# adeyemiadeoye/SelfConcordantSmoothOptimization.jl

Measured on AMD Instinct MI355X. Metric: iterate!() iterations/sec + achieved HBM GB/s, ProxGGNSCORE n=1M m=16k, higher is better.
Workload: dtype f64

## Files before the change

selfconcordantsmoothoptimization.jl_amd/csrc/gram.hip:

```cpp
#include <algorithm>
#include <cstdlib>
#include <type_traits>
#include <vector>

#include "common.h"

namespace scs {

}
#include "gram_strip.h"
namespace scs {

#define LDS_BARRIER()                                          \
  do {                                                         \
    asm volatile("s_waitcnt lgkmcnt(0)" ::: "memory");         \
    __builtin_amdgcn_s_barrier();                              \
    asm volatile("" ::: "memory");                             \
  } while (0)

__device__ __forceinline__ int bnd_claim(unsigned* ctr, int ntiles) {
  const int q8 = ntiles / 8, r8 = ntiles % 8;
  const int x0 = (int)((unsigned)__builtin_amdgcn_s_getreg((15 << 11) | 20) & 7u);
  for (int d = 0; d < 8; ++d) {
    const int x = (x0 + d) & 7, len = q8 + (x < r8 ? 1 : 0);
    if (len == 0) continue;
    const unsigned t = atomicAdd(ctr + x, 1u);
    if ((int)t < len) return x * q8 + (x < r8 ? x : r8) + (int)t;
  }
  return ntiles;
}
__device__ __forceinline__ int bnd_first(unsigned* ctr, unsigned skip, int ntiles, int* s) {
  if (threadIdx.x == 0) {
    const unsigned cu = ((unsigned)__builtin_amdgcn_s_getreg((31 << 11) | 4) >> 8) & 15u;
    const unsigned xcc = (unsigned)__builtin_amdgcn_s_getreg((15 << 11) | 20) & 7u;
    const unsigned xm = skip >> 24;
    const bool here = ((skip >> cu) & 1u) && (xm == 0 || ((xm >> xcc) & 1u));
    const unsigned arr = atomicAdd(ctr + 8, 1u);
    *s = (here && arr + 1 < gridDim.x) ? -1 : bnd_claim(ctr, ntiles);
  }
  __syncthreads();
  return *s;
}
__device__ __forceinline__ int bnd_next(unsigned* ctr, int ntiles, int* s) {
  __syncthreads();
  if (threadIdx.x == 0) *s = bnd_claim(ctr, ntiles);
  __syncthreads();
  return *s;
}

template <int TJC = 2>
__device__ __forceinline__ void gram_tile_store_row(const v4d (&acc)[4], int ti, int wr, int wc, int g, int fl,
                                                    int part, double* P, int GTI, int packed, int upper,
                                                    int accumulate, double* G, int64_t ldg, int tix, int bi, int bj) {
  auto addr = [&](int tj, int r) -> double* {
    const int il = wr * 64 + 16 * ti + g + 4 * r;
    const int jl = wc * 64 + 16 * tj + fl;
    if (part >= 0) return P + ((int64_t)part * GT + jl) * GTI + il;
    if (packed) return G + ((int64_t)tix * (GTI / GT) + il / GT) * GT * GT + jl * GT + (il % GT);
    if (upper) return G + ((int64_t)bi * GTI + il) * ldg + (int64_t)bj * GT + jl;
    return G + ((int64_t)bj * GT + jl) * ldg + (int64_t)bi * GTI + il;
  };
  if (accumulate && part < 0) {
#pragma unroll
// ... 404 lines not shown
  return hipGetLastError();
}

void gram_tile_list(int nb, int2* out, int* ntiles) {
  const int S = 8;
  const int nsb = (nb + S - 1) / S;
  int t = 0;
  for (int sbi = 0; sbi < nsb; ++sbi)
    for (int sbj = 0; sbj <= sbi; ++sbj)
      for (int i = sbi * S; i < (sbi + 1) * S && i < nb; ++i)
        for (int j = sbj * S; j < (sbj + 1) * S && j < nb; ++j)
          if (i >= j) out[t++] = make_int2(i, j);
  *ntiles = t;
}

void gram_tile_list_tall(int nb, int2* out, int* ntiles) {
  const int nbi = nb / 2, SI = 4, SJ = 8;
  int t = 0;
  for (int sbi = 0; sbi < (nbi + SI - 1) / SI; ++sbi)
    for (int sbj = 0; sbj <= sbi; ++sbj)
      for (int I = sbi * SI; I < (sbi + 1) * SI && I < nbi; ++I)
        for (int j = sbj * SJ; j < (sbj + 1) * SJ && j < nb; ++j)
          if (j <= 2 * I + 1) out[t++] = make_int2(I, j);
  *ntiles = t;
}

void gram_tile_list_rowmajor(int nb, int2* out) {
  int t = 0;
  for (int i = 0; i < nb; ++i)
    for (int j = 0; j <= i; ++j) out[t++] = make_int2(i, j);
}

hipError_t gram_launch_gen(const double* A1, int64_t lda1, const double* A2, int64_t lda2, const double* w,
                           int64_t k0, int64_t k1, const int2* tiles, int ntiles, double* G, int64_t ldg, int flags,
                           hipStream_t st);

template <int PIPE, int TI = 2, bool CM = false, bool AV = false, bool BND = false>
__global__ __launch_bounds__(128 * TI, (TI == 2 ? 2 : 1)) void gram_sia_kernel(
    const double* __restrict__ A, int64_t S, const double* __restrict__ w, int64_t k0, int64_t Nk,
    const int2* __restrict__ tiles, int ntiles, double* __restrict__ G, int64_t ldg, int flags,
    const int4* __restrict__ work, int seglen, int nsplit, double* __restrict__ P,
    const double* __restrict__ v, double* __restrict__ VP, int64_t vps, unsigned* __restrict__ scnt, int sob,
    const double* __restrict__ A2, int64_t S2) {
  static_assert(!(AV && CM), "the fused Aᵀv runs on the panel-blocked A only");
  constexpr int GTI = 64 * TI;
  constexpr int NT = 128 * TI;
  constexpr int FS = NT / 8;
  constexpr int NTI = 4;
  constexpr int NA = GTI / FS;
  constexpr int NB = GT / FS;
  constexpr int NMM = 2 * NTI * 4;
  constexpr int NRD = NTI + 4;
  constexpr int TAIL = NMM / 4;
  const int packed = flags & GRAM_PACKED, accumulate = flags & GRAM_ACCUMULATE, upper = flags & GRAM_UPPER;
  __shared__ __attribute__((aligned(16))) double lds[(GTI + GT) * GBK];
  const int orig = blockIdx.x;
  const int xcd = orig % 8;
  int bi, bj, tix, part = -1, piece = 0;
  __shared__ int s_claim;
  if constexpr (BND) {
    tix = bnd_first(scnt, (unsigned)sob, ntiles, &s_claim);
    if (tix < 0 || tix >= ntiles) return;
    bi = tiles[tix].x;
    bj = tiles[tix].y;
  } else if (work) {
    const int4 it = work[xcd * seglen + orig / 8];
    if (it.x < 0) return;
    bi = it.x;
    bj = it.y;
    tix = it.w;
    if (it.z >= 0) {
      piece = it.z;
      const int64_t L = ((Nk - k0 + (int64_t)nsplit * GBK - 1) / ((int64_t)nsplit * GBK)) * GBK;
      part = it.w;
      k0 = k0 + it.z * L;
      Nk = k0 + L < Nk ? k0 + L : Nk;
      if (Nk < k0) Nk = k0;
    }
  } else {
    const int q8 = ntiles / 8, r8 = ntiles % 8;
    tix = (xcd < r8 ? xcd * (q8 + 1) : r8 * (q8 + 1) + (xcd - r8) * q8) + orig / 8;
    const int2 tl = tiles[tix];
    bi = tl.x;
    bj = tl.y;
  }
bnd_tile:
  int tid_ = threadIdx.x;
  if constexpr (BND) asm volatile("" : "+v"(tid_));
  const int tid = tid_, lane = tid & 63, wid = tid >> 6;
  const int wr = wid >> 1, wc = wid & 1;
  const int sc = tid & 7, sf0 = tid >> 3;
  const int64_t st0 = k0 / GBK;
  const double* srcA = CM ? A + ((int64_t)bi * GTI + sf0) * S + k0 + 2 * sc
                          : A + ((int64_t)bi * (GTI / GT) * S + st0) * GT * GBK + sf0 * GBK + 2 * sc;
  const double* B2 = (CM && A2) ? A2 : A;
  const int64_t SB2 = (CM && A2) ? S2 : S;
  const double* srcB = CM ? B2 + ((int64_t)bj * GT + sf0) * SB2 + k0 + 2 * sc
                          : A + ((int64_t)bj * S + st0) * GT * GBK + sf0 * GBK + 2 * sc;
  const double* srcW = w + k0 + 2 * sc;
  const double* srcV = AV ? v + k0 + 2 * sc : nullptr;
  double* la = lds;
  double* lb = lds + GTI * GBK;
  int woff[NA];
#pragma unroll
  for (int i = 0; i < NA; ++i) {
    const int f = sf0 + FS * i;
    woff[i] = f * GBK + 2 * (sc ^ swz(f));
  }
  v2d ra[NA], rb[NB], rw, rv;
  double av[NB];
#pragma unroll
  for (int i = 0; i < NB; ++i) av[i] = 0.0;
  auto gload = [&](int64_t st, auto fa) {
    constexpr bool FA = decltype(fa)::value;
    if (PIPE == 3 && st >= 2) return;
    if (CM) {
#pragma unroll
      for (int i = 0; i < NA; ++i) ra[i] = *(const v2d*)(srcA + st * GBK + (int64_t)FS * i * S);
#pragma unroll
      for (int i = 0; i < NB; ++i) rb[i] = *(const v2d*)(srcB + st * GBK + (int64_t)FS * i * SB2);
    } else {
      const int64_t so = st * GT * GBK;
#pragma unroll
      for (int i = 0; i < NA; ++i) {
        const int f = FS * i;
        ra[i] = *(const v2d*)(srcA + so + (f >> 7) * S * GT * GBK + (f & 127) * GBK);
      }
#pragma unroll
      for (int i = 0; i < NB; ++i) rb[i] = *(const v2d*)(srcB + so + FS * GBK * i);
    }
    rw = *(const v2d*)(srcW + st * GBK);
    if (FA) rv = *(const v2d*)(srcV + st * GBK);
  };
  auto swrite = [&](auto fa) {
    constexpr bool FA = decltype(fa)::value;
#pragma unroll
    for (int i = 0; i < NA; ++i) *(v2d*)(la + woff[i]) = ra[i];
#pragma unroll
    for (int i = 0; i < NB; ++i) *(v2d*)(lb + woff[i]) = rb[i] * rw;
    if (FA) {
#pragma unroll
      for (int i = 0; i < NB; ++i) av[i] = __builtin_fma(rb[i][1], rv[1], __builtin_fma(rb[i][0], rv[0], av[i]));
    }
  };
  const int fl = lane & 15, g = lane >> 4, s = swz(fl);
  struct Frag {
    v2d a[NTI], b[4];
  };
  auto fread = [&](int p, Frag& F) {
    const int pc = ((4 * p + g) ^ s) * 2;
#pragma unroll
    for (int t = 0; t < NTI; ++t) F.a[t] = *(const v2d*)(la + (wr * 64 + 16 * t + fl) * GBK + pc);
#pragma unroll
    for (int t = 0; t < 4; ++t) F.b[t] = *(const v2d*)(lb + (wc * 64 + 16 * t + fl) * GBK + pc);
  };
  v4d acc[NTI][4];
#pragma unroll
  for (int i = 0; i < NTI; ++i)
#pragma unroll
    for (int j = 0; j < 4; ++j) acc[i][j] = (v4d){0.0, 0.0, 0.0, 0.0};
  auto mm = [&](const Frag& F, int n0, int n1) {
#pragma unroll
    for (int n = n0; n < n1; ++n) {
      const int u = n / (4 * NTI), ti = (n / 4) % NTI, tj = n & 3;
      acc[ti][tj] = __builtin_amdgcn_mfma_f64_16x16x4f64(F.a[ti][u], F.b[tj][u], acc[ti][tj], 0, 0, 0);
    }
  };
  auto barrier = [&]() {
    __builtin_amdgcn_sched_barrier(0);
    __builtin_amdgcn_s_waitcnt(0xC07F);
    __builtin_amdgcn_s_barrier();
    asm volatile("" ::: "memory");
    __builtin_amdgcn_sched_barrier(0);
  };
  const int nk = (int)((Nk - k0) / GBK);
  Frag F0, F1;
  auto run = [&](auto fa) {
    if (nk > 0) {
      gload(0, fa);
      swrite(fa);
      if (nk > 1) gload(1, fa);
      barrier();
      fread(0, F0);
    }
    auto body = [&](int k, bool has1, bool has2) {
      __builtin_amdgcn_sched_barrier(0);
      fread(1, F1);
      mm(F0, 0, NMM);
      if (PIPE) {
#pragma unroll
        for (int i = 0; i < NRD; ++i) {
          __builtin_amdgcn_sched_group_barrier(0x008, NMM / NRD, 0);
          __builtin_amdgcn_sched_group_barrier(0x100, 1, 0);
        }
      }
      barrier();
      if (has1) swrite(fa);
      if (has2) gload(k + 2, fa);
      mm(F1, 0, NMM - TAIL);
      if (PIPE) {
        if (has1) {
#pragma unroll
          for (int i = 0; i < NA + NB; ++i) {
            __builtin_amdgcn_sched_group_barrier(0x008, (NMM - TAIL) / (NA + NB), 0);
            __builtin_amdgcn_sched_group_barrier(0x200, 1, 0);
            if (has2) __builtin_amdgcn_sched_group_barrier(0x020, 1, 0);
          }
        }
        __builtin_amdgcn_sched_group_barrier(0x008, NMM, 0);
      }
      if (has1) {
        barrier();
        fread(0, F0);
      }
      mm(F1, NMM - TAIL, NMM);
      if (PIPE && has1) {
#pragma unroll
        for (int i = 0; i < NRD; ++i) {
          __builtin_amdgcn_sched_group_barrier(0x008, TAIL / NRD > 0 ? TAIL / NRD : 1, 0);
          __builtin_amdgcn_sched_group_barrier(0x100, 1, 0);
        }
      }
    };
    int k = 0;
    for (; k + 2 < nk; ++k) body(k, true, true);
    if (k + 1 < nk) {
      body(k, true, false);
      ++k;
    }
    if (k < nk) body(k, false, false);
  };
  const bool dav = AV && (int64_t)bj * GT / GTI == bi;
  if constexpr (AV) {
    if (dav) run(std::true_type{});
    else run(std::false_type{});
  } else {
    run(std::false_type{});
  }

  if (dav) {
#pragma unroll
    for (int i = 0; i < NB; ++i) {
      double t = av[i];
      t += __shfl_xor(t, 1);
      t += __shfl_xor(t, 2);
      t += __shfl_xor(t, 4);
      if (sc == 0) VP[(int64_t)piece * vps + (int64_t)bj * GT + sf0 + FS * i] = t;
    }
  }

  if constexpr (BND || CM) {
#pragma unroll
    for (int ti = 0; ti < NTI; ++ti)
      gram_tile_store_row(acc[ti], ti, wr, wc, g, fl, part, P, GTI, packed, upper, accumulate, G, ldg, tix, bi, bj);
  } else {
#pragma unroll
    for (int ti = 0; ti < NTI; ++ti)
#pragma unroll
      for (int tj = 0; tj < 4; ++tj)
#pragma unroll
        for (int r = 0; r < 4; ++r) {
          const int il = wr * 64 + 16 * ti + g + 4 * r;
          const int jl = wc * 64 + 16 * tj + fl;
          double* dst;
          if (part >= 0) {
            P[((int64_t)part * GT + jl) * GTI + il] = acc[ti][tj][r];
            continue;
          }
          if (packed) dst = G + ((int64_t)tix * (GTI / GT) + il / GT) * GT * GT + jl * GT + (il % GT);
          else if (upper) dst = G + ((int64_t)bi * GTI + il) * ldg + (int64_t)bj * GT + jl;
          else dst = G + ((int64_t)bj * GT + jl) * ldg + (int64_t)bi * GTI + il;
          if (accumulate) *dst += acc[ti][tj][r];
          else *dst = acc[ti][tj][r];
        }
  }
  if (!BND && scnt && part < 0) {
    __threadfence();
    __syncthreads();
    if (tid == 0) atomicAdd(scnt + bj / sob, 1u);
  }
  if constexpr (BND) {
    tix = bnd_next(scnt, ntiles, &s_claim);
    if (tix >= ntiles) return;
    bi = tiles[tix].x;
    bj = tiles[tix].y;
    goto bnd_tile;
  }
}

static int env_int(const char* name, int dflt) {
  const char* e = getenv(name);
  return e ? atoi(e) : dflt;
}
int gram_sia_mode() {
  static const int v = env_int("SCS_GRAM_SIA", 1);
  return v;
}
int gram_tall_mode() {
  static const int v = env_int("SCS_GRAM_GLDS", 3);
  return v;
}

int gram_fuse_ok(int tall) {
  const char* e = getenv("SCS_GRAM_FUSE");
  const int mode = e ? atoi(e) : 1;
  if (mode == 0 || (!tall && mode < 2)) return 0;
  return tall ? gram_tall_mode() == 3 : gram_sia_mode() == 1;
}

__global__ void gram_vfinal_kernel(const double* __restrict__ VP, int npiece, int64_t vps, int64_t m,
                                   double* __restrict__ out) {
  const int64_t f = (int64_t)blockIdx.x * blockDim.x + threadIdx.x;
  if (f >= m) return;
  double s = VP[f];
  for (int p = 1; p < npiece; ++p) s += VP[(int64_t)p * vps + f];
  out[f] = s;
}

hipError_t gram_vfinal_launch(const double* VP, int npiece, int64_t vps, int64_t m, double* out, hipStream_t st) {
  hipLaunchKernelGGL(gram_vfinal_kernel, dim3((unsigned)((m + 255) / 256)), dim3(256), 0, st, VP, npiece, vps, m, out);
  return hipGetLastError();
}

static thread_local const char* g_main_name = "";
const char* gram_main_kernel_name() { return g_main_name; }

hipError_t gram_launch(const double* A, int64_t lda, const double* w, int64_t Nk, const int2* tiles,
                       int ntiles, double* G, int64_t ldg, int packed, int tall, hipStream_t st, const double* v,
                       double* VP, int64_t vps) {
  if (ntiles <= 0) return hipSuccess;
  const int flags = ((packed & 1) ? GRAM_PACKED : GRAM_UPPER) | ((packed & 2) ? GRAM_ACCUMULATE : 0);
  if (v) {
    if (!gram_fuse_ok(tall)) return hipErrorInvalidValue;
    if (tall) {
      g_main_name = "gram_sia_kernel<1, 4, false, true, false>";
      hipLaunchKernelGGL((gram_sia_kernel<1, 4, false, true>), dim3(ntiles), dim3(512), 0, st, A, lda, w, (int64_t)0,
                         Nk, tiles, ntiles, G, ldg, flags, nullptr, 0, 0, nullptr, v, VP, vps, nullptr, 0, nullptr, (int64_t)0);
    } else {
      g_main_name = "gram_sia_kernel<1, 2, false, true, false>";
      hipLaunchKernelGGL((gram_sia_kernel<1, 2, false, true>), dim3(ntiles), dim3(256), 0, st, A, lda, w, (int64_t)0,
                         Nk, tiles, ntiles, G, ldg, flags, nullptr, 0, 0, nullptr, v, VP, vps, nullptr, 0, nullptr, (int64_t)0);
    }
    return hipGetLastError();
  }
  if (!tall && gram_sia_mode() == 0) {
    g_main_name = "gram_f64_kernel<false, 2, true, false>";
    hipLaunchKernelGGL((gram_f64_kernel<false, 2, true>), dim3(ntiles), dim3(256), 0, st, A, lda, A, lda, w,
                       (int64_t)0, Nk, tiles, ntiles, G, ldg, flags, nullptr, 0, 0, nullptr);
  } else if (!tall) {
    g_main_name = "gram_sia_kernel<1, 2, false, false, false>";
    hipLaunchKernelGGL((gram_sia_kernel<1, 2>), dim3(ntiles), dim3(256), 0, st, A, lda, w, (int64_t)0, Nk, tiles,
                       ntiles, G, ldg, flags, nullptr, 0, 0, nullptr, nullptr, nullptr, (int64_t)0, nullptr, 0, nullptr, (int64_t)0);
  } else if (gram_tall_mode() == 3) {
    g_main_name = "gram_sia_kernel<1, 4, false, false, false>";
    hipLaunchKernelGGL((gram_sia_kernel<1, 4>), dim3(ntiles), dim3(512), 0, st, A, lda, w, (int64_t)0, Nk, tiles,
                       ntiles, G, ldg, flags, nullptr, 0, 0, nullptr, nullptr, nullptr, (int64_t)0, nullptr, 0, nullptr, (int64_t)0);
  } else {
    g_main_name = "gram_glds_kernel<true, 1>";
    hipLaunchKernelGGL((gram_glds_kernel<true, 1>), dim3(ntiles), dim3(512), 0, st, A, lda, A, lda, w, (int64_t)0, Nk,
                       tiles, ntiles, G, ldg, flags, nullptr, 0, 0, nullptr);
  }
  return hipGetLastError();
}

template <int QC>
__global__ __launch_bounds__(256) void gram_small_kernel(const double* __restrict__ A1, int64_t lda1,
                                                         const double* A2, int64_t lda2,
                                                         const double* __restrict__ w, int64_t k0, int64_t Nk,
                                                         const int2* __restrict__ tiles, double* G, int64_t ldg,
                                                         int flags) {
  constexpr int NQ = GT / QC;
  __shared__ __attribute__((aligned(16))) double lds[2 * (GT + QC) * GBK];
  if (flags & GRAM_PRIO) __builtin_amdgcn_s_setprio(3);
  const int2 tl = tiles[blockIdx.x / NQ];
  const int64_t I0 = (int64_t)tl.x * GT, J0 = (int64_t)tl.y * GT + (blockIdx.x % NQ) * QC;
  double* Gt = (flags & GRAM_UPPER) ? G + I0 * ldg + J0 : G + J0 * ldg + I0;
  gram_small_strip<QC>(A1 + I0 * lda1, lda1, A2 + J0 * lda2, lda2, w, k0, Nk, Gt, ldg, flags, lds);
}

hipError_t gram_launch_small(const double* A1, int64_t lda1, const double* A2, int64_t lda2, const double* w,
                             int64_t k0, int64_t k1, const int2* tiles, int ntiles, double* G, int64_t ldg, int flags,
                             hipStream_t st) {
  if (ntiles <= 0) return hipSuccess;
  if ((k1 - k0) % (8 * GBK) != 0 || k1 <= k0) return hipErrorInvalidValue;
// ... 63 lines not shown
    hipLaunchKernelGGL((gram_sia_kernel<1, 2, true, false, true>), dim3(grid), dim3(256), 0, st, A1, lda1, w, k0, k1,
                       tiles, ntiles, G, ldg, flags, nullptr, 0, 0, nullptr, nullptr, nullptr, (int64_t)0, ctr,
                       (int)skip, nullptr, (int64_t)0);
  else if (gram_sia2(k1 - k0, lda2))
    hipLaunchKernelGGL((gram_sia_kernel<1, 2, true, false, true>), dim3(grid), dim3(256), 0, st, A1, lda1, w, k0, k1,
                       tiles, ntiles, G, ldg, flags, nullptr, 0, 0, nullptr, nullptr, nullptr, (int64_t)0, ctr,
                       (int)skip, A2, lda2);
  else
    hipLaunchKernelGGL((gram_f64_kernel<false, 2, false, true>), dim3(grid), dim3(256), 0, st, A1, lda1, A2, lda2, w,
                       k0, k1, tiles, ntiles, G, ldg, flags, nullptr, (int)skip, 0, reinterpret_cast<double*>(ctr));
  return hipGetLastError();
}

hipError_t gram_launch_ex(const double* A, int64_t lda, const double* w, int64_t k0, int64_t k1, const int2* tiles,
                          int ntiles, double* G, int64_t ldg, int accumulate, int noload, hipStream_t st) {
  const int flags = GRAM_UPPER | (accumulate ? GRAM_ACCUMULATE : 0);
  if (noload == 16 || noload == 17)
    hipLaunchKernelGGL((noload == 16 ? gram_sia_kernel<1, 4> : gram_sia_kernel<3, 4>), dim3(ntiles), dim3(512), 0,
                       st, A, (k1 - k0) / GBK, w, k0, k1, tiles, ntiles, G, ldg, flags, nullptr, 0, 0, nullptr, nullptr, nullptr, (int64_t)0, nullptr, 0, nullptr, (int64_t)0);
  else if (noload == 12)
    hipLaunchKernelGGL((gram_sia_kernel<3>), dim3(ntiles), dim3(256), 0, st, A, (k1 - k0) / GBK, w, k0, k1, tiles,
                       ntiles, G, ldg, flags, nullptr, 0, 0, nullptr, nullptr, nullptr, (int64_t)0, nullptr, 0, nullptr, (int64_t)0);
  else if (noload == 9 || noload == 10)
    hipLaunchKernelGGL((noload == 9 ? gram_sia_kernel<1> : gram_sia_kernel<0>), dim3(ntiles), dim3(256), 0, st, A,
                       (k1 - k0) / GBK, w, k0, k1, tiles, ntiles, G, ldg, flags, nullptr, 0, 0, nullptr, nullptr, nullptr, (int64_t)0, nullptr, 0, nullptr, (int64_t)0);
  else if (noload == 11)
    hipLaunchKernelGGL((gram_f64_kernel<false, 2, true>), dim3(ntiles), dim3(256), 0, st, A, (k1 - k0) / GBK, A,
                       (k1 - k0) / GBK, w, k0, k1, tiles, ntiles, G, ldg, flags, nullptr, 0, 0, nullptr);
  else if (noload == 7 || noload == 8)
    hipLaunchKernelGGL((noload == 7 ? gram_glds_kernel<true, 1> : gram_glds_kernel<true, 2>), dim3(ntiles), dim3(512),
                       0, st, A, (k1 - k0) / GBK, A, (k1 - k0) / GBK, w, k0, k1, tiles, ntiles, G, ldg, flags, nullptr,
                       0, 0, nullptr);
  else if (noload == 5)
    hipLaunchKernelGGL(gram_glds_kernel<true>, dim3(ntiles), dim3(512), 0, st, A, (k1 - k0) / GBK, A,
                       (k1 - k0) / GBK, w, k0, k1, tiles, ntiles, G, ldg, flags, nullptr, 0, 0, nullptr);
  else if (noload == 6)
    hipLaunchKernelGGL(gram_glds_kernel<false>, dim3(ntiles), dim3(512), 0, st, A, lda, A, lda, w, k0, k1, tiles,
                       ntiles, G, ldg, flags, nullptr, 0, 0, nullptr);
  else if (noload == 4)
    hipLaunchKernelGGL((gram_f64_kernel<true, 4>), dim3(ntiles), dim3(512), 0, st, A, lda, A, lda, w, k0, k1, tiles,
                       ntiles, G, ldg, flags, nullptr, 0, 0, nullptr);
  else if (noload == 3)
    hipLaunchKernelGGL((gram_f64_kernel<false, 4>), dim3(ntiles), dim3(512), 0, st, A, lda, A, lda, w, k0, k1, tiles,
                       ntiles, G, ldg, flags, nullptr, 0, 0, nullptr);
  else if (noload)
    hipLaunchKernelGGL((gram_f64_kernel<true, 2>), dim3(ntiles), dim3(256), 0, st, A, lda, A, lda, w, k0, k1, tiles,
                       ntiles, G, ldg, flags, nullptr, 0, 0, nullptr);
  else
    hipLaunchKernelGGL((gram_f64_kernel<false, 2>), dim3(ntiles), dim3(256), 0, st, A, lda, A, lda, w, k0, k1, tiles,
                       ntiles, G, ldg, flags, nullptr, 0, 0, nullptr);
  return hipGetLastError();
}

template <int TI>
__global__ void gram_combine_kernel(const double* __restrict__ P, const int4* __restrict__ items, int nsplit,
                                    double* __restrict__ G, int64_t ldg, int packed) {
  constexpr int GTI = 64 * TI;
  const int4 it = items[blockIdx.y];
  for (int e = blockIdx.x * blockDim.x + threadIdx.x; e < GTI * GT; e += gridDim.x * blockDim.x) {
    const int jl = e / GTI, il = e % GTI;
    double sum = 0.0;
    for (int sp = 0; sp < nsplit; ++sp) sum += P[(int64_t)(it.w + sp) * GTI * GT + e];
    double* dst = (packed & 1) ? G + ((int64_t)it.z * (GTI / GT) + il / GT) * GT * GT + jl * GT + (il % GT)
                               : G + ((int64_t)it.x * GTI + il) * ldg + (int64_t)it.y * GT + jl;
    if (packed & 2) *dst += sum;
    else *dst = sum;
  }
}

hipError_t gram_launch_sched(const double* A, int64_t lda, const double* w, int64_t Nk, const int4* work, int seglen,
                             int nsplit, const int4* comb, int ncomb, double* P, double* G, int64_t ldg, int packed,
                             int tall, hipStream_t st, const double* v, double* VP, int64_t vps, unsigned* scnt,
                             int sob) {
  if (scnt && !(gram_fuse_ok(tall) || (tall ? gram_tall_mode() == 3 : gram_sia_mode() == 1)))
    return hipErrorInvalidValue;
  const int flags = ((packed & 1) ? GRAM_PACKED : GRAM_UPPER) | ((packed & 2) ? GRAM_ACCUMULATE : 0);
  const int glds = gram_tall_mode();
  if (v && !gram_fuse_ok(tall)) return hipErrorInvalidValue;
  if (v && tall) {
    g_main_name = "gram_sia_kernel<1, 4, false, true, false>";
    hipLaunchKernelGGL((gram_sia_kernel<1, 4, false, true>), dim3(8 * seglen), dim3(512), 0, st, A, lda, w,
                       (int64_t)0, Nk, nullptr, 0, G, ldg, flags, work, seglen, nsplit, P, v, VP, vps, scnt, sob, nullptr, (int64_t)0);
  } else if (v) {
    g_main_name = "gram_sia_kernel<1, 2, false, true, false>";
    hipLaunchKernelGGL((gram_sia_kernel<1, 2, false, true>), dim3(8 * seglen), dim3(256), 0, st, A, lda, w,
                       (int64_t)0, Nk, nullptr, 0, G, ldg, flags, work, seglen, nsplit, P, v, VP, vps, scnt, sob, nullptr, (int64_t)0);
  } else if (tall && glds == 3) {
    g_main_name = "gram_sia_kernel<1, 4, false, false, false>";
    hipLaunchKernelGGL((gram_sia_kernel<1, 4>), dim3(8 * seglen), dim3(512), 0, st, A, lda, w, (int64_t)0, Nk,
                       nullptr, 0, G, ldg, flags, work, seglen, nsplit, P, nullptr, nullptr, (int64_t)0, scnt, sob, nullptr, (int64_t)0);
  } else if (tall && glds == 2) {
    g_main_name = "gram_glds_kernel<true, 1>";
    hipLaunchKernelGGL((gram_glds_kernel<true, 1>), dim3(8 * seglen), dim3(512), 0, st, A, lda, A, lda, w, (int64_t)0,
                       Nk, nullptr, 0, G, ldg, flags, work, seglen, nsplit, P);
  } else if (tall && glds == 1) {
    g_main_name = "gram_glds_kernel<true, 0>";
    hipLaunchKernelGGL(gram_glds_kernel<true>, dim3(8 * seglen), dim3(512), 0, st, A, lda, A, lda, w, (int64_t)0, Nk,
                       nullptr, 0, G, ldg, flags, work, seglen, nsplit, P);
  } else if (tall) {
    g_main_name = "gram_f64_kernel<false, 4, true, false>";
    hipLaunchKernelGGL((gram_f64_kernel<false, 4, true>), dim3(8 * seglen), dim3(512), 0, st, A, lda, A, lda, w,
                       (int64_t)0, Nk, nullptr, 0, G, ldg, flags, work, seglen, nsplit, P);
  } else if (gram_sia_mode() == 1) {
    g_main_name = "gram_sia_kernel<1, 2, false, false, false>";
    hipLaunchKernelGGL((gram_sia_kernel<1, 2>), dim3(8 * seglen), dim3(256), 0, st, A, lda, w, (int64_t)0, Nk, nullptr,
                       0, G, ldg, flags, work, seglen, nsplit, P, nullptr, nullptr, (int64_t)0, scnt, sob, nullptr, (int64_t)0);
  } else if (gram_sia_mode() == 2) {
    g_main_name = "gram_sia_kernel<0, 2, false, false, false>";
    hipLaunchKernelGGL((gram_sia_kernel<0>), dim3(8 * seglen), dim3(256), 0, st, A, lda, w, (int64_t)0, Nk, nullptr, 0,
                       G, ldg, flags, work, seglen, nsplit, P, nullptr, nullptr, (int64_t)0, scnt, sob, nullptr, (int64_t)0);
  } else {
    g_main_name = "gram_f64_kernel<false, 2, true, false>";
    hipLaunchKernelGGL((gram_f64_kernel<false, 2, true>), dim3(8 * seglen), dim3(256), 0, st, A, lda, A, lda, w,
                       (int64_t)0, Nk, nullptr, 0, G, ldg, flags, work, seglen, nsplit, P);
  }
  if (ncomb > 0) {
    if (tall)
      hipLaunchKernelGGL(gram_combine_kernel<4>, dim3(16, ncomb), dim3(256), 0, st, P, comb, nsplit, G, ldg, packed);
    else
      hipLaunchKernelGGL(gram_combine_kernel<2>, dim3(16, ncomb), dim3(256), 0, st, P, comb, nsplit, G, ldg, packed);
  }
  return hipGetLastError();
}

__global__ void strip_wait_kernel(const unsigned* __restrict__ cnt, unsigned target, int* __restrict__ flag) {
  if (threadIdx.x != 0) return;
  const uint64_t t0 = __builtin_amdgcn_s_memrealtime();
  while (__hip_atomic_load(cnt, __ATOMIC_ACQUIRE, __HIP_MEMORY_SCOPE_AGENT) < target) {
    __builtin_amdgcn_s_sleep(16);
    if (__builtin_amdgcn_s_memrealtime() - t0 > 3000000000ull) {
      __hip_atomic_store(flag, 1, __ATOMIC_RELAXED, __HIP_MEMORY_SCOPE_AGENT);
      break;
    }
  }
}

hipError_t strip_wait_launch(const unsigned* cnt, unsigned target, int* flag, hipStream_t st) {
  hipLaunchKernelGGL(strip_wait_kernel, dim3(1), dim3(64), 0, st, cnt, target, flag);
  return hipGetLastError();
}

hipError_t gram_launch_sched_cm(const double* X, int64_t ld, const double* w, int64_t k0, int64_t k1, const int4* work,
                                int seglen, int nsplit, const int4* comb, int ncomb, double* P, double* G, int64_t ldg,
                                int flags, hipStream_t st) {
  if (seglen <= 0 || k1 <= k0) return hipSuccess;
  hipLaunchKernelGGL((gram_sia_kernel<1, 2, true>), dim3(8 * seglen), dim3(256), 0, st, X, ld, w, k0, k1, nullptr, 0,
                     G, ldg, flags | GRAM_UPPER, work, seglen, nsplit, P, nullptr, nullptr, (int64_t)0, nullptr, 0, nullptr, (int64_t)0);
  if (ncomb > 0)
    hipLaunchKernelGGL(gram_combine_kernel<2>, dim3(16, ncomb), dim3(256), 0, st, P, comb, nsplit, G, ldg,
                       (flags & GRAM_ACCUMULATE) ? 2 : 0);
  return hipGetLastError();
}

int gram_schedule(const int2* tiles, int ntiles, int slots_per_xcd, std::vector<int4>& work, std::vector<int4>& comb,
                  int* nsplit, int* npart, int diag_first_gti) {
  const int q = ntiles / 8, r = ntiles % 8;
  int tail_max = 0;
  for (int x = 0; x < 8; ++x) {
    const int n = q + (x < r ? 1 : 0);
    const int t = n % slots_per_xcd;
    tail_max = std::max(tail_max, t);
  }
  int S = 1;
  if (tail_max > 0 && 4 * tail_max < 3 * slots_per_xcd)
    S = std::max(2, std::min(16, slots_per_xcd / tail_max));
  std::vector<std::vector<int4>> seg(8);
  comb.clear();
  int pslot = 0, t0 = 0;
  for (int x = 0; x < 8; ++x) {
    const int n = q + (x < r ? 1 : 0);
    const int tail = (S > 1) ? n % slots_per_xcd : 0;
    for (int i = 0; i < n - tail; ++i) {
      const int2 tl = tiles[t0 + i];
      seg[x].push_back(make_int4(tl.x, tl.y, -1, t0 + i));
    }
    if (diag_first_gti > 0)
      std::stable_partition(seg[x].begin(), seg[x].end(), [&](const int4& it) {
        return it.x == (int)((int64_t)it.y * GT / diag_first_gti);
      });
    for (int i = n - tail; i < n; ++i) {
      const int2 tl = tiles[t0 + i];
      comb.push_back(make_int4(tl.x, tl.y, t0 + i, pslot));
      for (int sp = 0; sp < S; ++sp) seg[x].push_back(make_int4(tl.x, tl.y, sp, pslot + sp));
      pslot += S;
    }
    t0 += n;
  }
  size_t seglen = 0;
  for (auto& v : seg) seglen = std::max(seglen, v.size());
  work.assign(8 * seglen, make_int4(-1, -1, -1, -1));
  for (int x = 0; x < 8; ++x)
    for (size_t i = 0; i < seg[x].size(); ++i) work[x * seglen + i] = seg[x][i];
  *nsplit = S;
  *npart = pslot;
  return (int)seglen;
}

hipError_t gram_unpack_launch(const double* P, const int2* tiles, int ntiles, double* G, int64_t ldg,
                              hipStream_t st) {
  if (ntiles <= 0) return hipSuccess;
  hipLaunchKernelGGL(gram_packx_kernel<true>, dim3(4, ntiles), dim3(256), 0, st, P, G, tiles, ldg);
  return hipGetLastError();
}

}
```

selfconcordantsmoothoptimization.jl_amd/csrc/gram_strip.h:

```cpp
#pragma once
#include "common.h"

namespace scs {

constexpr int GT = 128;
enum { GRAM_PACKED = 1, GRAM_ACCUMULATE = 2, GRAM_UPPER = 4, GRAM_PRIO = 8 };
constexpr int GBK = 16;

__device__ __forceinline__ int swz(int f) { return (f >> 1) & 7; }

template <int TJ>
__device__ __forceinline__ void gram_strip_store(const v4d (&acc)[2][TJ], double* Gt, int64_t ldg, int wr, int g,
                                                 int fl, int accumulate, int upper) {
  double* dst[2][TJ][4];
#pragma unroll
  for (int ti = 0; ti < 2; ++ti)
#pragma unroll
    for (int tj = 0; tj < TJ; ++tj)
#pragma unroll
      for (int r = 0; r < 4; ++r) {
        const int64_t I = wr * 32 + 16 * ti + g + 4 * r;
        const int64_t J = 16 * tj + fl;
        dst[ti][tj][r] = upper ? Gt + I * ldg + J : Gt + J * ldg + I;
      }
  if (accumulate) {
    double old[2][TJ][4];
#pragma unroll
    for (int ti = 0; ti < 2; ++ti)
#pragma unroll
      for (int tj = 0; tj < TJ; ++tj)
#pragma unroll
        for (int r = 0; r < 4; ++r) old[ti][tj][r] = *dst[ti][tj][r];
#pragma unroll
    for (int ti = 0; ti < 2; ++ti)
#pragma unroll
      for (int tj = 0; tj < TJ; ++tj)
#pragma unroll
        for (int r = 0; r < 4; ++r) *dst[ti][tj][r] = old[ti][tj][r] + acc[ti][tj][r];
  } else {
#pragma unroll
    for (int ti = 0; ti < 2; ++ti)
#pragma unroll
      for (int tj = 0; tj < TJ; ++tj)
#pragma unroll
        for (int r = 0; r < 4; ++r) *dst[ti][tj][r] = acc[ti][tj][r];
  }
}

template <int QC>
__device__ __forceinline__ void gram_small_strip(const double* __restrict__ Ai, int64_t lda1, const double* Aj,
                                                 int64_t lda2, const double* __restrict__ w, int64_t k0, int64_t Nk,
                                                 double* Gt, int64_t ldg, int flags, double* lds) {
  constexpr int RING = 8;
  constexpr int NQ = GT / QC;
  constexpr int TJ = QC / 16;
  constexpr int SBQ = (GT + QC) * GBK;
  (void)NQ;
  const int accumulate = flags & GRAM_ACCUMULATE, upper = flags & GRAM_UPPER;
  const int tid = threadIdx.x, lane = tid & 63, wr = tid >> 6;
// ... 63 lines not shown
```

selfconcordantsmoothoptimization.jl_amd/csrc/kernels.h:

```cpp
#pragma once
#include <hip/hip_runtime.h>
#include <stdint.h>

#include <vector>
#include "../../include/scsopt.h"

namespace scs {

struct ProxArgsH {
  int reg = 0;
  int use_prox = 1;
  double lam = 0.0, lam2 = 0.0;
  const double* lb = nullptr;
  const double* ub = nullptr;
  const int* gstart = nullptr;
  const int* gend = nullptr;
  const double* gw = nullptr;
  int ngroups = 0;
  const int* gmap = nullptr;
};

void gram_tile_list(int nb, int2* out, int* ntiles);
void gram_tile_list_tall(int nb, int2* out, int* ntiles);
const char* gram_main_kernel_name();
hipError_t gram_launch(const double* A, int64_t lda, const double* w, int64_t Nk, const int2* tiles, int ntiles,
                       double* G, int64_t ldg, int packed, int tall, hipStream_t st, const double* v = nullptr,
                       double* VP = nullptr, int64_t vps = 0);
int gram_fuse_ok(int tall);
hipError_t gram_vfinal_launch(const double* VP, int npiece, int64_t vps, int64_t m, double* out, hipStream_t st);
void gram_tile_list_rowmajor(int nb, int2* out);
hipError_t gram_launch_gen(const double* A1, int64_t lda1, const double* A2, int64_t lda2, const double* w,
                           int64_t k0, int64_t k1, const int2* tiles, int ntiles, double* G, int64_t ldg, int flags,
                           hipStream_t st);
hipError_t gram_launch_work_cm(const double* A1, int64_t lda1, const double* A2, int64_t lda2, const double* w,
                               int64_t K, const int4* work, int seglen, int nsplit, double* P, hipStream_t st);
hipError_t gram_launch_bounded(const double* A1, int64_t lda1, const double* A2, int64_t lda2, const double* w,
                               int64_t k0, int64_t k1, const int2* tiles, int ntiles, double* G, int64_t ldg, int flags,
                               unsigned* ctr, unsigned skip, int slots, hipStream_t st, bool zeroed = false);
hipError_t gram_launch_small(const double* A1, int64_t lda1, const double* A2, int64_t lda2, const double* w,
                             int64_t k0, int64_t k1, const int2* tiles, int ntiles, double* G, int64_t ldg, int flags,
                             hipStream_t st);
int gram_schedule(const int2* tiles, int ntiles, int slots_per_xcd, std::vector<int4>& work, std::vector<int4>& comb,
                  int* nsplit, int* npart, int diag_first_gti = 0);
hipError_t gram_launch_sched(const double* A, int64_t lda, const double* w, int64_t Nk, const int4* work, int seglen,
                             int nsplit, const int4* comb, int ncomb, double* P, double* G, int64_t ldg, int packed,
                             int tall, hipStream_t st, const double* v = nullptr, double* VP = nullptr,
                             int64_t vps = 0, unsigned* scnt = nullptr, int sob = 0);
hipError_t strip_wait_launch(const unsigned* cnt, unsigned target, int* flag, hipStream_t st);
hipError_t gram_pack_launch(const double* G, int64_t ldg, const int2* tiles, int ntiles, double* P, hipStream_t st);
hipError_t gram_unpack_launch(const double* P, const int2* tiles, int ntiles, double* G, int64_t ldg,
                              hipStream_t st);

struct DagTask {
  int64_t a1, a2, out;
  int32_t lda1, a1w;
  int32_t k0, nk;
  int32_t wneg, flags;
  int32_t dep0, ndep;
  int32_t sig0, sig1;
};
struct DagDep {
  int32_t c, target;
};
struct DagList {
  int t0 = 0, nt = 0;
  unsigned gen = 0;
};

struct CholAux {
  double* w = nullptr;
  int2* rect = nullptr;
  hipStream_t st2 = nullptr;
  hipStream_t stc = nullptr;
  hipStream_t st2h = nullptr;
  hipEvent_t ev1 = nullptr, ev2 = nullptr, ev3 = nullptr, ev4 = nullptr, ev0 = nullptr, ev5 = nullptr;
  int nblk = 0;
  unsigned* bctr = nullptr;
  int2* sbl = nullptr;
  unsigned bskip = 0;
  int bslots = 0;
  mutable int bslot = 0;
  mutable int chain_mode = 0;
  double* sscr = nullptr;
  struct StripSched {
    int4* work = nullptr;
    int seglen = 0, nsplit = 1;
    int4* comb = nullptr;
    int ncomb = 0;
  };
  std::vector<StripSched> ssched;
  double* spart = nullptr;
  unsigned* sflags = nullptr;
  int* serr = nullptr;
  unsigned sgen = 0;
  mutable bool no_persist = false;
  mutable bool no_dag = false;
// ... 235 lines not shown
```

selfconcordantsmoothoptimization.jl_amd/csrc/scsopt.cpp:

```cpp
#include <hip/hip_runtime.h>
#include <rccl/rccl.h>

#include <dlfcn.h>
#include <execinfo.h>
#include <signal.h>

#include <algorithm>
#include <chrono>
#include <cmath>
#include <cstdarg>
#include <cstddef>
#include <cstdio>
#include <cstdlib>
#include <cstring>
#include <limits>
#include <atomic>
#include <condition_variable>
#include <functional>
#include <memory>
#include <mutex>
#include <string>
#include <thread>
#include <utility>
#include <vector>
// ... 545 lines not shown
  c->nval = epilogue_blocks(c->Npad);
  c->nchunk = c->sparse ? c->bcsc.nblk : gemv_t_chunks(c->Npad);
  dfree_t(c, c->zpart);
  dfree_t(c, c->z);
  dfree_t(c, c->gN);
  dfree_t(c, c->hN);
  dfree_t(c, c->wN);
  dfree_t(c, c->vN);
  dfree_t(c, c->valpart);
  dfree_t(c, c->tpart);
  c->zpart = dalloc<double>(c, (size_t)c->nsplit * c->Npad);
  c->z = dalloc<double>(c, c->Npad);
  c->gN = dalloc<double>(c, c->Npad);
  c->hN = dalloc<double>(c, c->Npad);
  c->wN = dalloc<double>(c, c->Npad);
  c->vN = dalloc<double>(c, c->Npad);
  c->valpart = dalloc<double>(c, c->nval);
  c->tpart = dalloc<double>(c, (size_t)c->nchunk * c->mpad);
}

void ensure_gram(scs_ctx* c) {
  if (c->G) return;
  const int64_t mp = c->mpad;
  c->G = dalloc<double>(c, (size_t)mp * mp);
  c->Gc = dalloc<double>(c, (size_t)mp * mp);
  const int nb = (int)(mp / 128);
  std::vector<int2> tl((size_t)nb * (nb + 1) / 2 + nb), ul;
  int nt = 0;
  const char* sq = std::getenv("SCS_GRAM_TALL");
  c->tall = (nb % 2 == 0) && nb >= 96 && !(sq && sq[0] == '0');
  if (sq && sq[0] == '1') c->tall = (nb % 2 == 0);
  if (c->tall) {
    gram_tile_list_tall(nb, tl.data(), &nt);
    ul.resize(2 * (size_t)nt);
    for (int t = 0; t < nt; ++t) {
      ul[2 * t] = make_int2(2 * tl[t].x, tl[t].y);
      ul[2 * t + 1] = make_int2(2 * tl[t].x + 1, tl[t].y);
    }
  } else {
    gram_tile_list(nb, tl.data(), &nt);
    ul.assign(tl.begin(), tl.begin() + nt);
  }
  c->tiles = dalloc<int2>(c, nt);
  HCK(hipMemcpyAsync(c->tiles, tl.data(), sizeof(int2) * nt, hipMemcpyHostToDevice, c->st));
  c->ntiles = nt;
  c->nslots = (int)ul.size();
  {
    const char* ev = std::getenv("SCS_GRAM_SCHED");
    if (!(ev && ev[0] == '0')) {
      std::vector<int4> wk, cb;
      int npart = 0;
      const char* df = std::getenv("SCS_GRAM_DIAGFIRST");
      const int dfg = (df && df[0] == '0') ? 0 : c->tall ? 256 : (df && df[0] == '1') ? 128 : 0;
      c->gseglen = gram_schedule(tl.data(), nt, 32 * (c->tall ? 1 : 2), wk, cb, &c->gnsplit, &npart, dfg);
      c->gncomb = (int)cb.size();
      c->gwork = dalloc<int4>(c, wk.size());
      HCK(hipMemcpyAsync(c->gwork, wk.data(), sizeof(int4) * wk.size(), hipMemcpyHostToDevice, c->st));
      if (c->gncomb > 0) {
        c->gcomb = dalloc<int4>(c, cb.size());
        HCK(hipMemcpyAsync(c->gcomb, cb.data(), sizeof(int4) * cb.size(), hipMemcpyHostToDevice, c->st));
        c->gpart = dalloc<double>(c, (size_t)npart * (c->tall ? 256 : 128) * 128);
      }
    }
  }
  {
    const int OB = chol_outer_block(), ns = (nb + OB - 1) / OB;
    c->gstrip.assign(ns, scs_ctx::GStrip());
    c->vpieces = std::max(c->gnsplit, 1);
    int npart_max = 0;
    for (int s2 = 0; s2 < ns; ++s2) {
      std::vector<int2> st;
      for (int t = 0; t < nt; ++t)
        if (tl[t].y / OB == s2) st.push_back(tl[t]);
      std::vector<int4> wk, cb;
      int nsplit = 1, npart = 0;
      scs_ctx::GStrip& g = c->gstrip[s2];
      g.seglen = gram_schedule(st.data(), (int)st.size(), 32 * (c->tall ? 1 : 2), wk, cb, &nsplit, &npart);
      g.nsplit = nsplit;
      g.ncomb = (int)cb.size();
      g.work = dalloc<int4>(c, wk.size());
      HCK(hipMemcpyAsync(g.work, wk.data(), sizeof(int4) * wk.size(), hipMemcpyHostToDevice, c->st));
      if (!cb.empty()) {
        g.comb = dalloc<int4>(c, cb.size());
        HCK(hipMemcpyAsync(g.comb, cb.data(), sizeof(int4) * cb.size(), hipMemcpyHostToDevice, c->st));
      }
      npart_max = std::max(npart_max, npart);
      c->vpieces = std::max(c->vpieces, nsplit);
    }
    {
      const int slots = 32 * (c->tall ? 1 : 2);
      std::vector<std::vector<int4>> seg(8);
      c->gp_target.assign(ns, 0u);
      std::vector<int4> cbl;
      int nsplit = 1, npart = 0;
      for (int s2 = 0; s2 < ns; ++s2) {
        std::vector<int2> st;
        std::vector<int> ix;
        for (int t = 0; t < nt; ++t)
          if (tl[t].y / OB == s2) {
            st.push_back(tl[t]);
            ix.push_back(t);
          }
        const int n = (int)st.size();
        if (s2 + 1 < ns) {
          c->gp_target[s2] = (unsigned)n;
          const int q = n / 8, r = n % 8;
          int t0 = 0;
// ... 3589 lines not shown
```

Measured before the change: 0.2560.

## Skip redundant lower-half MFMA work on symmetric diagonal Gram tiles in tall mode

In the tall (TI=4) Gram kernel, tiles where bj == 2*bi+1 straddle the diagonal, so half of the 256x128 output block is a redundant copy of the other half. For those tiles the waves covering that half (wid<4) now skip their LDS fragment reads and MFMAs but still take part in global loads, LDS writes and barriers, and the A-panel rows shared with B are not reloaded. The host scheduler is reworked to place these cheaper tiles separately and spread them evenly across XCDs. Correctness relies on the epilogue mirroring or ignoring the skipped half, which is not visible here.

Measured after the change: 0.2580, median of 6. No clear change (+0.8%).

```diff
diff --git a/selfconcordantsmoothoptimization.jl_amd/csrc/gram.hip b/selfconcordantsmoothoptimization.jl_amd/csrc/gram.hip
--- a/selfconcordantsmoothoptimization.jl_amd/csrc/gram.hip
+++ b/selfconcordantsmoothoptimization.jl_amd/csrc/gram.hip
@@ -9,6 +9,7 @@
 
 }
 #include "gram_strip.h"
+#include "gram_schedule.h"
 namespace scs {
 
 #define LDS_BARRIER()                                          \
@@ -519,6 +520,8 @@
   constexpr int NMM = 2 * NTI * 4;
   constexpr int NRD = NTI + 4;
   constexpr int TAIL = NMM / 4;
+  constexpr int NA0 = GT / FS;
+  constexpr bool SYMM_OK = TI == 4 && !CM && !BND;
   const int packed = flags & GRAM_PACKED, accumulate = flags & GRAM_ACCUMULATE, upper = flags & GRAM_UPPER;
   __shared__ __attribute__((aligned(16))) double lds[(GTI + GT) * GBK];
   const int orig = blockIdx.x;
@@ -578,18 +581,19 @@
   double av[NB];
 #pragma unroll
   for (int i = 0; i < NB; ++i) av[i] = 0.0;
-  auto gload = [&](int64_t st, auto fa) {
+  auto gload = [&](int64_t st, auto fa, auto dt) {
     constexpr bool FA = decltype(fa)::value;
+    constexpr int IA0 = decltype(dt)::value ? NA0 : 0;
     if (PIPE == 3 && st >= 2) return;
     if (CM) {
 #pragma unroll
-      for (int i = 0; i < NA; ++i) ra[i] = *(const v2d*)(srcA + st * GBK + (int64_t)FS * i * S);
+      for (int i = IA0; i < NA; ++i) ra[i] = *(const v2d*)(srcA + st * GBK + (int64_t)FS * i * S);
 #pragma unroll
       for (int i = 0; i < NB; ++i) rb[i] = *(const v2d*)(srcB + st * GBK + (int64_t)FS * i * SB2);
     } else {
       const int64_t so = st * GT * GBK;
 #pragma unroll
-      for (int i = 0; i < NA; ++i) {
+      for (int i = IA0; i < NA; ++i) {
         const int f = FS * i;
         ra[i] = *(const v2d*)(srcA + so + (f >> 7) * S * GT * GBK + (f & 127) * GBK);
       }
@@ -599,10 +603,11 @@
     rw = *(const v2d*)(srcW + st * GBK);
     if (FA) rv = *(const v2d*)(srcV + st * GBK);
   };
-  auto swrite = [&](auto fa) {
+  auto swrite = [&](auto fa, auto dt) {
     constexpr bool FA = decltype(fa)::value;
-#pragma unroll
-    for (int i = 0; i < NA; ++i) *(v2d*)(la + woff[i]) = ra[i];
+    constexpr int IA0 = decltype(dt)::value ? NA0 : 0;
+#pragma unroll
+    for (int i = IA0; i < NA; ++i) *(v2d*)(la + woff[i]) = ra[i];
 #pragma unroll
     for (int i = 0; i < NB; ++i) *(v2d*)(lb + woff[i]) = rb[i] * rw;
     if (FA) {
@@ -642,19 +647,23 @@
   };
   const int nk = (int)((Nk - k0) / GBK);
   Frag F0, F1;
-  auto run = [&](auto fa) {
+  auto run = [&](auto fa, auto dt, auto dw) {
+    constexpr bool LIVE = !decltype(dw)::value;
+    constexpr int NAW = decltype(dt)::value ? NA - NA0 : NA;
     if (nk > 0) {
-      gload(0, fa);
-      swrite(fa);
-      if (nk > 1) gload(1, fa);
+      gload(0, fa, dt);
+      swrite(fa, dt);
+      if (nk > 1) gload(1, fa, dt);
       barrier();
-      fread(0, F0);
+      if (LIVE) fread(0, F0);
     }
     auto body = [&](int k, bool has1, bool has2) {
       __builtin_amdgcn_sched_barrier(0);
-      fread(1, F1);
-      mm(F0, 0, NMM);
-      if (PIPE) {
+      if (LIVE) {
+        fread(1, F1);
+        mm(F0, 0, NMM);
+      }
+      if (PIPE && LIVE) {
 #pragma unroll
         for (int i = 0; i < NRD; ++i) {
           __builtin_amdgcn_sched_group_barrier(0x008, NMM / NRD, 0);
@@ -662,14 +671,14 @@
         }
       }
       barrier();
-      if (has1) swrite(fa);
-      if (has2) gload(k + 2, fa);
-      mm(F1, 0, NMM - TAIL);
-      if (PIPE) {
+      if (has1) swrite(fa, dt);
+      if (has2) gload(k + 2, fa, dt);
+      if (LIVE) mm(F1, 0, NMM - TAIL);
+      if (PIPE && LIVE) {
         if (has1) {
 #pragma unroll
-          for (int i = 0; i < NA + NB; ++i) {
-            __builtin_amdgcn_sched_group_barrier(0x008, (NMM - TAIL) / (NA + NB), 0);
+          for (int i = 0; i < NAW + NB; ++i) {
+            __builtin_amdgcn_sched_group_barrier(0x008, (NMM - TAIL) / (NAW + NB), 0);
             __builtin_amdgcn_sched_group_barrier(0x200, 1, 0);
             if (has2) __builtin_amdgcn_sched_group_barrier(0x020, 1, 0);
           }
@@ -678,10 +687,10 @@
       }
       if (has1) {
         barrier();
-        fread(0, F0);
+        if (LIVE) fread(0, F0);
       }
-      mm(F1, NMM - TAIL, NMM);
-      if (PIPE && has1) {
+      if (LIVE) mm(F1, NMM - TAIL, NMM);
+      if (PIPE && LIVE && has1) {
 #pragma unroll
         for (int i = 0; i < NRD; ++i) {
           __builtin_amdgcn_sched_group_barrier(0x008, TAIL / NRD > 0 ? TAIL / NRD : 1, 0);
@@ -698,11 +707,24 @@
     if (k < nk) body(k, false, false);
   };
   const bool dav = AV && (int64_t)bj * GT / GTI == bi;
-  if constexpr (AV) {
-    if (dav) run(std::true_type{});
-    else run(std::false_type{});
-  } else {
-    run(std::false_type{});
+  constexpr std::true_type T{};
+  constexpr std::false_type F{};
+  bool dtop = false;
+  if constexpr (SYMM_OK) {
+    dtop = (flags & GRAM_SYMM) && bj == 2 * bi + 1;
+    if (dtop) {
+      constexpr std::bool_constant<AV> fa{};
+      if (__builtin_amdgcn_readfirstlane(wid) < 4) run(fa, T, T);
+      else run(fa, T, F);
+    }
+  }
+  if (!dtop) {
+    if constexpr (AV) {
+      if (dav) run(T, F, F);
+      else run(F, F, F);
+    } else {
+      run(F, F, F);
+    }
   }
 
   if (dav) {
@@ -775,6 +797,11 @@
   return tall ? gram_tall_mode() == 3 : gram_sia_mode() == 1;
 }
 
+int gram_symm_ok() {
+  const char* e = getenv("SCS_GRAM_SYMM");
+  return !(e && e[0] == '0');
+}
+
 __global__ void gram_vfinal_kernel(const double* __restrict__ VP, int npiece, int64_t vps, int64_t m,
                                    double* __restrict__ out) {
   const int64_t f = (int64_t)blockIdx.x * blockDim.x + threadIdx.x;
@@ -796,7 +823,8 @@
                        int ntiles, double* G, int64_t ldg, int packed, int tall, hipStream_t st, const double* v,
                        double* VP, int64_t vps) {
   if (ntiles <= 0) return hipSuccess;
-  const int flags = ((packed & 1) ? GRAM_PACKED : GRAM_UPPER) | ((packed & 2) ? GRAM_ACCUMULATE : 0);
+  const int flags = ((packed & 1) ? GRAM_PACKED : GRAM_UPPER) | ((packed & 2) ? GRAM_ACCUMULATE : 0) |
+                    ((tall && gram_symm_ok()) ? GRAM_SYMM : 0);
   if (v) {
     if (!gram_fuse_ok(tall)) return hipErrorInvalidValue;
     if (tall) {
@@ -966,6 +994,14 @@
   return hipGetLastError();
 }
 
+hipError_t gram_launch_symm_ex(const double* A, int64_t S, const double* w, int64_t Nk, const int2* tiles, int ntiles,
+                               double* G, int64_t ldg, int symm, const double* v, double* VP, hipStream_t st) {
+  hipLaunchKernelGGL((gram_sia_kernel<1, 4, false, true>), dim3(ntiles), dim3(512), 0, st, A, S, w, (int64_t)0, Nk,
+                     tiles, ntiles, G, ldg, GRAM_UPPER | (symm ? GRAM_SYMM : 0), nullptr, 0, 0, nullptr, v, VP,
+                     (int64_t)0, nullptr, 0, nullptr, (int64_t)0);
+  return hipGetLastError();
+}
+
 template <int TI>
 __global__ void gram_combine_kernel(const double* __restrict__ P, const int4* __restrict__ items, int nsplit,
                                     double* __restrict__ G, int64_t ldg, int packed) {
@@ -988,7 +1024,8 @@
                              int sob) {
   if (scnt && !(gram_fuse_ok(tall) || (tall ? gram_tall_mode() == 3 : gram_sia_mode() == 1)))
     return hipErrorInvalidValue;
-  const int flags = ((packed & 1) ? GRAM_PACKED : GRAM_UPPER) | ((packed & 2) ? GRAM_ACCUMULATE : 0);
+  const int flags = ((packed & 1) ? GRAM_PACKED : GRAM_UPPER) | ((packed & 2) ? GRAM_ACCUMULATE : 0) |
+                    ((tall && gram_symm_ok()) ? GRAM_SYMM : 0);
   const int glds = gram_tall_mode();
   if (v && !gram_fuse_ok(tall)) return hipErrorInvalidValue;
   if (v && tall) {
@@ -1067,47 +1104,8 @@
 }
 
 int gram_schedule(const int2* tiles, int ntiles, int slots_per_xcd, std::vector<int4>& work, std::vector<int4>& comb,
-                  int* nsplit, int* npart, int diag_first_gti) {
-  const int q = ntiles / 8, r = ntiles % 8;
-  int tail_max = 0;
-  for (int x = 0; x < 8; ++x) {
-    const int n = q + (x < r ? 1 : 0);
-    const int t = n % slots_per_xcd;
-    tail_max = std::max(tail_max, t);
-  }
-  int S = 1;
-  if (tail_max > 0 && 4 * tail_max < 3 * slots_per_xcd)
-    S = std::max(2, std::min(16, slots_per_xcd / tail_max));
-  std::vector<std::vector<int4>> seg(8);
-  comb.clear();
-  int pslot = 0, t0 = 0;
-  for (int x = 0; x < 8; ++x) {
-    const int n = q + (x < r ? 1 : 0);
-    const int tail = (S > 1) ? n % slots_per_xcd : 0;
-    for (int i = 0; i < n - tail; ++i) {
-      const int2 tl = tiles[t0 + i];
-      seg[x].push_back(make_int4(tl.x, tl.y, -1, t0 + i));
-    }
-    if (diag_first_gti > 0)
-      std::stable_partition(seg[x].begin(), seg[x].end(), [&](const int4& it) {
-        return it.x == (int)((int64_t)it.y * GT / diag_first_gti);
-      });
-    for (int i = n - tail; i < n; ++i) {
-      const int2 tl = tiles[t0 + i];
-      comb.push_back(make_int4(tl.x, tl.y, t0 + i, pslot));
-      for (int sp = 0; sp < S; ++sp) seg[x].push_back(make_int4(tl.x, tl.y, sp, pslot + sp));
-      pslot += S;
-    }
-    t0 += n;
-  }
-  size_t seglen = 0;
-  for (auto& v : seg) seglen = std::max(seglen, v.size());
-  work.assign(8 * seglen, make_int4(-1, -1, -1, -1));
-  for (int x = 0; x < 8; ++x)
-    for (size_t i = 0; i < seg[x].size(); ++i) work[x * seglen + i] = seg[x][i];
-  *nsplit = S;
-  *npart = pslot;
-  return (int)seglen;
+                  int* nsplit, int* npart, int diag_first_gti, double cheap_cost) {
+  return gram_schedule_t(tiles, ntiles, slots_per_xcd, work, comb, nsplit, npart, diag_first_gti, cheap_cost, GT);
 }
 
 hipError_t gram_unpack_launch(const double* P, const int2* tiles, int ntiles, double* G, int64_t ldg,
diff --git a/selfconcordantsmoothoptimization.jl_amd/csrc/gram_schedule.h b/selfconcordantsmoothoptimization.jl_amd/csrc/gram_schedule.h
--- /dev/null
+++ b/selfconcordantsmoothoptimization.jl_amd/csrc/gram_schedule.h
@@ -0,0 +1,74 @@
+#pragma once
+#include <algorithm>
+#include <vector>
+
+namespace scs {
+
+constexpr double GRAM_HALF_COST = 0.52;
+
+template <class I2, class I4>
+int gram_schedule_t(const I2* tiles, int ntiles, int slots_per_xcd, std::vector<I4>& work, std::vector<I4>& comb,
+                    int* nsplit, int* npart, int diag_first_gti = 0, double cheap_cost = 1.0, int gt = 128) {
+  auto item = [](int x, int y, int z, int w) {
+    I4 it;
+    it.x = x;
+    it.y = y;
+    it.z = z;
+    it.w = w;
+    return it;
+  };
+  std::vector<std::vector<int>> idx(8);
+  int nfull[8];
+  std::vector<int> full, cheap;
+  const bool by_cost = cheap_cost > 0.0 && cheap_cost < 1.0;
+  for (int t = 0; t < ntiles; ++t) (by_cost && tiles[t].y == 2 * tiles[t].x + 1 ? cheap : full).push_back(t);
+  {
+    const int q = (int)full.size() / 8, r = (int)full.size() % 8;
+    const int qc = (int)cheap.size() / 8, rc = (int)cheap.size() % 8;
+    int t0 = 0, c0 = 0;
+    for (int x = 0; x < 8; ++x) {
+      const int n = q + (x < r ? 1 : 0);
+      const int nc = qc + (x >= 8 - rc ? 1 : 0);
+      idx[x].assign(full.begin() + t0, full.begin() + t0 + n);
+      idx[x].insert(idx[x].end(), cheap.begin() + c0, cheap.begin() + c0 + nc);
+      nfull[x] = n;
+      t0 += n;
+      c0 += nc;
+    }
+  }
+  int tail_max = 0;
+  for (int x = 0; x < 8; ++x) tail_max = std::max(tail_max, (int)idx[x].size() % slots_per_xcd);
+  int S = 1;
+  if (tail_max > 0 && 4 * tail_max < 3 * slots_per_xcd) S = std::max(2, std::min(16, slots_per_xcd / tail_max));
+  std::vector<std::vector<I4>> seg(8);
+  comb.clear();
+  int pslot = 0;
+  for (int x = 0; x < 8; ++x) {
+    const int n = (int)idx[x].size();
+    const int tail = (S > 1) ? n % slots_per_xcd : 0;
+    for (int i = 0; i < n - tail; ++i) {
+      const I2 tl = tiles[idx[x][i]];
+      seg[x].push_back(item(tl.x, tl.y, -1, idx[x][i]));
+    }
+    if (diag_first_gti > 0)
+      std::stable_partition(seg[x].begin(), seg[x].begin() + std::min(n - tail, nfull[x]), [&](const I4& it) {
+        return it.x == (int)((long long)it.y * gt / diag_first_gti);
+      });
+    for (int i = n - tail; i < n; ++i) {
+      const I2 tl = tiles[idx[x][i]];
+      comb.push_back(item(tl.x, tl.y, idx[x][i], pslot));
+      for (int sp = 0; sp < S; ++sp) seg[x].push_back(item(tl.x, tl.y, sp, pslot + sp));
+      pslot += S;
+    }
+  }
+  size_t seglen = 0;
+  for (auto& v : seg) seglen = std::max(seglen, v.size());
+  work.assign(8 * seglen, item(-1, -1, -1, -1));
+  for (int x = 0; x < 8; ++x)
+    for (size_t i = 0; i < seg[x].size(); ++i) work[x * seglen + i] = seg[x][i];
+  *nsplit = S;
+  *npart = pslot;
+  return (int)seglen;
+}
+
+}
diff --git a/selfconcordantsmoothoptimization.jl_amd/csrc/gram_strip.h b/selfconcordantsmoothoptimization.jl_amd/csrc/gram_strip.h
--- a/selfconcordantsmoothoptimization.jl_amd/csrc/gram_strip.h
+++ b/selfconcordantsmoothoptimization.jl_amd/csrc/gram_strip.h
@@ -4,7 +4,7 @@
 namespace scs {
 
 constexpr int GT = 128;
-enum { GRAM_PACKED = 1, GRAM_ACCUMULATE = 2, GRAM_UPPER = 4, GRAM_PRIO = 8 };
+enum { GRAM_PACKED = 1, GRAM_ACCUMULATE = 2, GRAM_UPPER = 4, GRAM_PRIO = 8, GRAM_SYMM = 16 };
 constexpr int GBK = 16;
 
 __device__ __forceinline__ int swz(int f) { return (f >> 1) & 7; }
diff --git a/selfconcordantsmoothoptimization.jl_amd/csrc/kernels.h b/selfconcordantsmoothoptimization.jl_amd/csrc/kernels.h
--- a/selfconcordantsmoothoptimization.jl_amd/csrc/kernels.h
+++ b/selfconcordantsmoothoptimization.jl_amd/csrc/kernels.h
@@ -4,6 +4,7 @@
 
 #include <vector>
 #include "../../include/scsopt.h"
+#include "gram_schedule.h"
 
 namespace scs {
 
@@ -41,7 +42,8 @@
                              int64_t k0, int64_t k1, const int2* tiles, int ntiles, double* G, int64_t ldg, int flags,
                              hipStream_t st);
 int gram_schedule(const int2* tiles, int ntiles, int slots_per_xcd, std::vector<int4>& work, std::vector<int4>& comb,
-                  int* nsplit, int* npart, int diag_first_gti = 0);
+                  int* nsplit, int* npart, int diag_first_gti = 0, double cheap_cost = 1.0);
+int gram_symm_ok();
 hipError_t gram_launch_sched(const double* A, int64_t lda, const double* w, int64_t Nk, const int4* work, int seglen,
                              int nsplit, const int4* comb, int ncomb, double* P, double* G, int64_t ldg, int packed,
                              int tall, hipStream_t st, const double* v = nullptr, double* VP = nullptr,
diff --git a/selfconcordantsmoothoptimization.jl_amd/csrc/scsopt.cpp b/selfconcordantsmoothoptimization.jl_amd/csrc/scsopt.cpp
--- a/selfconcordantsmoothoptimization.jl_amd/csrc/scsopt.cpp
+++ b/selfconcordantsmoothoptimization.jl_amd/csrc/scsopt.cpp
@@ -621,7 +621,8 @@
       int npart = 0;
       const char* df = std::getenv("SCS_GRAM_DIAGFIRST");
       const int dfg = (df && df[0] == '0') ? 0 : c->tall ? 256 : (df && df[0] == '1') ? 128 : 0;
-      c->gseglen = gram_schedule(tl.data(), nt, 32 * (c->tall ? 1 : 2), wk, cb, &c->gnsplit, &npart, dfg);
+      const double cheap = (c->tall && gram_symm_ok()) ? GRAM_HALF_COST : 1.0;
+      c->gseglen = gram_schedule(tl.data(), nt, 32 * (c->tall ? 1 : 2), wk, cb, &c->gnsplit, &npart, dfg, cheap);
       c->gncomb = (int)cb.size();
       c->gwork = dalloc<int4>(c, wk.size());
       HCK(hipMemcpyAsync(c->gwork, wk.data(), sizeof(int4) * wk.size(), hipMemcpyHostToDevice, c->st));
```
